# rchikhi/rust-seq2kminmers

Measured on AMD Instinct MI355X. Metric: input bases/s (Gbp/s) for k-min-mer extraction, l=31 k=10 d=0.01, higher is better.
Workload: dtype u32

## Files before the change

### rust-seq2kminmers_amd/csrc/s2k_api.hip

```cpp
#include "../../include/s2k.h"
#include "s2k_dev.h"
#include "s2k_hostcopy.h"

#include <math.h>
#include <stdio.h>
#include <stdlib.h>
#include <string.h>
#include <string>
#include <algorithm>
#include <atomic>
#include <chrono>
#include <condition_variable>
#include <thread>
#include <memory>
#include <mutex>
#include <sys/mman.h>
#include <vector>

using namespace s2k;

static_assert(offsetof(Counts, path) == offsetof(s2k_counts, path), "Counts must start with s2k_counts");

namespace {

// ... 516 lines not shown
                                  use_desc ? (unsigned long long *)d_agg : nullptr, agg_pack(0, 0, 0, 0, true, true), sp),
                "read table kernel");
        Sem sem = c.sem;
        sem.read_runs = nullptr;
        sem.tile_heads = nullptr;
        if (want_runs) {
            if (c.full_runs) {
                S2K_TRY(launch_read_run_counts(c.d_bases, c.d_read_off, n_reads, n_bases, run_blk, run_off, run_tmp, read_runs, nullptr, sp),
                        "run count kernels");
                sem.read_runs = read_runs;
            } else {
                S2K_TRY(hipMemsetAsync(tile_heads, 0, n_tiles * sizeof(uint32_t), sp), "memset tile head words");
                sem.tile_heads = tile_heads;
            }
        }
        if (use_desc) {
            Desc dz{};
            dz.agg = d_agg;
            dz.meta = d_meta;
            dz.state = d_state;
            dz.k = c.sem.k;
            dz.spec_n = ctx->rec_per_tile_hint ? ctx->rec_per_tile_hint : 192u;
            dz.km_capacity = o.km_capacity;
            dz.mn_capacity = o.mn_capacity;
            dz.o_km_off = (unsigned long long *)o.km_off;
            dz.o_hash = (unsigned long long *)o.hash;
            dz.o_start = o.start;
            dz.o_end = o.end;
            dz.o_rev = o.rev;
            dz.o_mn_off = (unsigned long long *)mn_off;
            dz.o_mn_j = o.mn_j;
            dz.o_mn_jend = o.mn_jend;
            dz.o_mn_hash = o.mn_hash;
            dz.xor_shards = (unsigned long long *)ctx->d_xor;
            if (tm) S2K_TRY(hipEventRecord(ctx->ev[1], sp), "event");
            if (tm && n_chunks > 1) S2K_TRY(hipEventRecord(ctx->ev[3], sk), "event");
            for (uint32_t ch = 0; ch < n_chunks; ch++) {
                auto cut = [&](uint32_t i) -> uint64_t {
                    static const double tail = getenv("S2K_DESC_TAIL") ? atof(getenv("S2K_DESC_TAIL")) : 0.0;
                    if (i >= n_chunks) return n_tiles;
                    if (tail <= 0.0 || tail >= 1.0 || n_chunks < 2) return n_tiles * i / n_chunks;
                    return (uint64_t)((double)n_tiles * (1.0 - tail) * (double)i / (double)(n_chunks - 1));
                };
                const uint64_t T0 = cut(ch), T1 = cut(ch + 1);
                const bool last = ch + 1 == n_chunks;
                S2K_TRY(launch_tile_minimizers(c.d_bases, c.d_read_off, n_reads, n_bases, T1, tile_read0, sem, rec,
                                               pool_cursor + (size_t)CURSOR_WORDS * ch, nullptr, nullptr, nullptr, ctx->d_counts, &dz, T0, sp),
                        "tiled minimizer kernel");
                if (last) {
                    S2K_TRY(hipEventRecord(ctx->tiles_done, sp), "event");
                    ctx->tiles_done_valid = true;
                    if (tm) S2K_TRY(hipEventRecord(ctx->ev[2], sp), "event");
                }
                S2K_TRY(hipEventRecord(ctx->chunk_ev[ch], sp), "event");
                S2K_TRY(hipStreamWaitEvent(sk, ctx->chunk_ev[ch], 0), "stream wait");
                if (tm && n_chunks == 1) S2K_TRY(hipEventRecord(ctx->ev[3], sk), "event");
#ifdef S2K_DEBUG_KNOBS
                static const bool nokm = getenv("S2K_DEBUG_NOKM") != nullptr;
                if (nokm) continue;
#endif
                S2K_TRY(launch_desc_scan(T0, T1, dz, d_scan, ctx->d_counts, sk), "tile word scan");
                S2K_TRY(launch_desc_kminmers(T0, T1, n_tiles, n_reads, dz, rec, ctx->d_counts, sk, last && !(chained && c.sem.hpc)), "k-min-mer kernel");
            }
            if (tm) S2K_TRY(hipEventRecord(ctx->ev[4], sk), "event");
            S2K_TRY(launch_finalize(ctx->d_counts, ctx->d_xor, (const uint64_t *)&d_state[n_tiles].gmn, (const uint64_t *)&d_state[n_tiles].g,
                                    o.km_capacity, o.mn_capacity, sk),
                    "finalize kernel");
            S2K_TRY(hipMemcpyAsync(ctx->h_counts, ctx->d_counts, sizeof(Counts), hipMemcpyDeviceToHost, sk), "counts copy");
            if (tm) S2K_TRY(hipEventRecord(ctx->ev[5], sk), "event");
            S2K_TRY(mark_done(ctx), "event");
            ctx->pending = true;
            return S2K_OK;
        }
        if (tm) S2K_TRY(hipEventRecord(ctx->ev[1], sp), "event");
        S2K_TRY(launch_tile_minimizers(c.d_bases, c.d_read_off, n_reads, n_bases, n_tiles, tile_read0, sem, rec, pool_cursor,
                                       tile_rec_off, tile_cnt, mn_cnt, ctx->d_counts, nullptr, 0, sp),
                "tiled minimizer kernel");
        s2k_status hs = hand_over();
        if (hs != S2K_OK) return hs;
        S2K_TRY(launch_scan_u32(tile_cnt, n_tiles, tile_goff, scan_tmp, 0, sk), "scan");
        S2K_TRY(launch_scan_u32(mn_cnt, n_reads, mn_off, scan_tmp, 0, sk), "scan");
    }
    S2K_TRY(launch_scan_u32(mn_cnt, n_reads, o.km_off, scan_tmp, c.sem.k, sk), "scan");
    if (tm) S2K_TRY(hipEventRecord(ctx->ev[3], sk), "event");
    S2K_TRY(launch_kminmers(n_tiles, tile_rec_off, tile_cnt, tile_goff, rec, mn_off, o.km_off, c.sem.k, o.km_capacity, o.hash,
                            o.start, o.end, o.rev, o.mn_capacity, o.mn_capacity ? o.mn_j : nullptr, o.mn_jend, o.mn_hash,
                            ctx->d_xor, ctx->d_counts, sk),
            "k-min-mer kernel");
    if (tm) S2K_TRY(hipEventRecord(ctx->ev[4], sk), "event");
    S2K_TRY(launch_finalize(ctx->d_counts, ctx->d_xor, mn_off + n_reads, o.km_off + n_reads, o.km_capacity, o.mn_capacity, sk),
// ... 808 lines not shown
```

### rust-seq2kminmers_amd/csrc/s2k_dev.h

```cpp
#pragma once
#include <hip/hip_runtime.h>
#include <stdint.h>

namespace s2k {

constexpr uint32_t SEED_A = 0x95c60474u, SEED_C = 0x62a02b4cu, SEED_G = 0x82572324u, SEED_T = 0x4be24456u;

__host__ __device__ inline uint32_t seed_h_scalar(uint32_t c) {
    return c == 'A' ? SEED_A : c == 'C' ? SEED_C : c == 'G' ? SEED_G : c == 'T' ? SEED_T : c == 'N' ? 0u : 1u;
}
__host__ __device__ inline uint32_t seed_rc_scalar(uint32_t c) {
    return c == 'A' ? SEED_T : c == 'C' ? SEED_G : c == 'G' ? SEED_C : c == 'T' ? SEED_A : c == 'N' ? 0u : 1u;
}
__host__ __device__ inline uint32_t seed_h_simd(uint32_t c) {
    uint32_t n = c & 15u;
    return n == 1 ? SEED_A : n == 3 ? SEED_C : n == 7 ? SEED_G : n == 4 ? SEED_T : 0u;
}
__host__ __device__ inline uint32_t seed_rc_simd(uint32_t c) {
    uint32_t n = c & 15u;
    return n == 1 ? SEED_T : n == 3 ? SEED_G : n == 7 ? SEED_C : n == 4 ? SEED_A : 0u;
}

#if defined(__HIP_DEVICE_COMPILE__)
__device__ __forceinline__ uint32_t xor3(uint32_t a, uint32_t b, uint32_t c) {
// ... 20 lines not shown
struct Sem {
    uint32_t l;
    uint32_t k;
    uint32_t bound_le;
    uint32_t enabled;
    uint32_t hpc;
    uint32_t simd_seeds;
    uint32_t keep_last;
    uint32_t end_kind;
    uint32_t tail_quirk;
    uint32_t dbg_skip;
    uint32_t pad_;
    const uint32_t *read_runs;
    uint32_t *tile_heads;
};

struct Counts {
    uint64_t n_reads, n_bases, n_minimizers, n_kminmers, xor_hash;
    uint32_t hash_bound, path;
    uint64_t pool_needed;
    uint32_t pool_overflow, bad_input, km_overflow, mn_overflow;
    uint32_t need_legacy, need_runs;
    uint64_t dbg_cycles[64][16];
#ifdef S2K_DEBUG_KNOBS
    uint64_t dbg_wave[4096][2];
#endif
};

constexpr uint32_t HW_VALID = 1u << 31, HW_PASS = 1u << 30, HW_COUNT = 0xFFFFu;

// ... 133 lines not shown

hipError_t launch_serial_count(const uint8_t *bases, const uint64_t *read_off, uint64_t n_reads, uint64_t n_bases, Sem sem,
                               uint32_t *mn_cnt, hipStream_t st);
hipError_t launch_serial_write(const uint8_t *bases, const uint64_t *read_off, uint64_t n_reads, uint64_t n_bases, Sem sem,
                               const uint64_t *mn_off, Records rec, Counts *counts, hipStream_t st);

hipError_t launch_kminmers(uint64_t n_tiles, const uint64_t *tile_rec_off, const uint32_t *tile_cnt,
                           const uint64_t *tile_goff, Records rec, const uint64_t *mn_off, const uint64_t *km_off,
                           uint32_t k, uint64_t km_capacity, uint64_t *o_hash, uint32_t *o_start, uint32_t *o_end,
                           uint8_t *o_rev, uint64_t mn_capacity, uint32_t *o_mn_j, uint32_t *o_mn_jend,
                           uint32_t *o_mn_hash, uint64_t *xor_shards, const Counts *counts, hipStream_t st);
hipError_t launch_finalize(Counts *counts, const uint64_t *xor_shards, const uint64_t *mn_total, const uint64_t *km_total,
                           uint64_t km_capacity, uint64_t mn_capacity, hipStream_t st);

hipError_t launch_tile_minimizers(const uint8_t *bases, const uint64_t *read_off, uint64_t n_reads, uint64_t n_bases,
                                  uint64_t n_tiles, const uint32_t *tile_read0, Sem sem, Records rec,
                                  uint64_t *pool_cursor, uint64_t *tile_rec_off, uint32_t *tile_cnt, uint32_t *mn_cnt,
                                  Counts *counts, const Desc *desc, uint64_t tile_begin, hipStream_t st);
hipError_t launch_desc_scan(uint64_t tile_begin, uint64_t tile_end, Desc dz, unsigned long long *scan_tmp ,
                            const Counts *counts, hipStream_t st);
size_t desc_scan_tmp_words(uint64_t n_tiles);
hipError_t launch_desc_kminmers(uint64_t tile_begin, uint64_t tile_end, uint64_t n_tiles, uint64_t n_reads, Desc dz, Records rec, Counts *counts,
                                hipStream_t st, bool alone);

hipError_t launch_hpc_count(const uint8_t *bases, const uint64_t *read_off, uint64_t n_reads, uint32_t *run_cnt, hipStream_t st,
                            bool rle = false);
hipError_t launch_hpc_write(const uint8_t *bases, const uint64_t *read_off, uint64_t n_reads, const uint64_t *hpc_off,
                            uint8_t *o_hpc, uint32_t *o_pos, uint64_t capacity, hipStream_t st, bool rle = false);

size_t fx_ws_bytes(uint64_t n);
hipError_t fx_parse_count(const uint8_t *d_raw, uint64_t n, int fastq, void *ws, uint64_t *d_totals, hipStream_t st);
// ... 5 lines not shown
```

### rust-seq2kminmers_amd/csrc/s2k_tile.hip

```cpp
#include "s2k_tile_impl.h"

namespace s2k {

#define S2K_DECL(LV)                                                                                                     \
    hipError_t launch_tiles_static_##LV(bool hpc, hipStream_t st, const uint8_t *bases, const uint64_t *read_off,         \
                                        uint64_t n_reads, uint64_t n_bases, uint64_t n_tiles, const uint32_t *tile_read0, \
                                        Sem sem, Records rec, uint64_t *pool_cursor, uint64_t *tile_rec_off,             \
                                        uint32_t *tile_cnt, uint32_t *mn_cnt, Counts *counts, const Desc *desc, uint64_t tile_begin);
S2K_STATIC_LS(S2K_DECL)
#undef S2K_DECL


hipError_t launch_tile_minimizers(const uint8_t *bases, const uint64_t *read_off, uint64_t n_reads, uint64_t n_bases,
                                  uint64_t n_tiles, const uint32_t *tile_read0, Sem sem, Records rec,
                                  uint64_t *pool_cursor, uint64_t *tile_rec_off, uint32_t *tile_cnt, uint32_t *mn_cnt,
                                  Counts *counts, const Desc *desc, uint64_t tile_begin, hipStream_t st) {
    if (n_tiles <= tile_begin || n_reads == 0) return hipSuccess;
    if (sem.l > (uint32_t)MAX_L_TILED || (sem.hpc && sem.tail_quirk && !sem.read_runs && !sem.tile_heads)) return hipErrorInvalidValue;
    if (desc && (desc->k == 0 || desc->k > 32u || !desc->agg || !desc->meta)) return hipErrorInvalidValue;
    switch (sem.l) {
#define S2K_CASE(LV)                                                                                                   \
    case LV:                                                                                                           \
        return launch_tiles_static_##LV(sem.hpc, st, bases, read_off, n_reads, n_bases, n_tiles, tile_read0, sem, rec, \
                                        pool_cursor, tile_rec_off, tile_cnt, mn_cnt, counts, desc, tile_begin);
        S2K_STATIC_LS(S2K_CASE)
#undef S2K_CASE
    default:
        return launch_tiles_l<0>(sem.hpc, st, bases, read_off, n_reads, n_bases, n_tiles, tile_read0, sem, rec,
                                 pool_cursor, tile_rec_off, tile_cnt, mn_cnt, counts, desc, tile_begin);
    }
}

}
```

### rust-seq2kminmers_amd/csrc/s2k_tile_impl.h

```cpp
#pragma once
#include "s2k_dev.h"
#include "s2k_static_l.h"

#include <cstdlib>
#include <mutex>
#include <type_traits>

namespace s2k {
namespace {

#ifndef S2K_TW
#define S2K_TW 12
#endif
#ifndef S2K_TW_REG
#ifdef S2K_PROFILE
#define S2K_TW_REG 12
#else
#define S2K_TW_REG 16
#endif
#endif
template <bool HPC> constexpr int tw() { return HPC ? S2K_TW : S2K_TW_REG; }
template <bool HPC> constexpr int waves_per_simd() { return tw<HPC>() / 4; }
static_assert(S2K_TW % 4 == 0 && S2K_TW_REG % 4 == 0, "whole waves per SIMD");
constexpr int HS_OFF = 16;
// ... 1061 lines not shown
                        f ^= rotl32(ti.x, l - 1 - i);
                        r ^= rotr32(ti.y, l - 1 - i);
                    }
                }
            }
            f ^= (uint32_t)__builtin_amdgcn_update_dpp(0, (int)f, 0xB1, 0xf, 0xf, false);
            r ^= (uint32_t)__builtin_amdgcn_update_dpp(0, (int)r, 0xB1, 0xf, 0xf, false);
            f ^= (uint32_t)__builtin_amdgcn_update_dpp(0, (int)f, 0x4E, 0xf, 0xf, false);
            r ^= (uint32_t)__builtin_amdgcn_update_dpp(0, (int)r, 0x4E, 0xf, 0xf, false);
            if (act && part == 0) rec.hash[base + S.jobslot[job]] = f < r ? f : r;
        }
        njobs = 0;
        wave_sync();
    };
    auto batch = [&](uint32_t b0, auto single_c) {
        constexpr bool SINGLE = decltype(single_c)::value;
        wave_sync();
        bool listed = false;
        if constexpr (HPC && SINGLE && S2K_LPH != 0) {
            if (Tq <= 112u) {
                listed = true;
                typedef __attribute__((address_space(3))) uint8_t lds_b;
                typedef __attribute__((address_space(3))) uint32_t lds_w;
                typedef uint32_t u32x2 __attribute__((ext_vector_type(2)));
                typedef uint32_t u32x4 __attribute__((ext_vector_type(4)));
                typedef __attribute__((address_space(3))) u32x2 lds_w2;
                typedef __attribute__((address_space(3))) u32x4 lds_w4;
                constexpr uint32_t XT = TILE_BASES + 128 - 2048;
                static_assert(XT % 16 == 0 && XT >= 7168 + MAX_L_TILED + 16 && LISTCAP <= 192, "the tables of the listing must not reach into the compacted tile");
                const uint32_t dq = (uint32_t)(uintptr_t)(lds_b *)const_cast<uint8_t *>(D) + XT;
// ... 62 lines not shown
#pragma unroll
            for (int d = 0; d < 5; d++) {
                uint32_t wv = vm[d];
                const uint32_t rw = raw[d];
                constexpr int CPW = 32 / CAPP;
                auto capw = [&](int i) { return caps[(CPW * d + i) < NPC ? CPW * d + i : NPC - 1]; };
                const uint32_t cap0 = capw(0), cap1 = capw(1), cap2 = capw(CPW > 2 ? 2 : 0), cap3 = capw(CPW > 2 ? 3 : 1);
                while (wv) {
                    const uint32_t bit = __builtin_ctz(wv);
                    wv &= wv - 1;
                    const uint32_t pm = CAPP == 16 ? (0xFFFFu << (bit & 16)) : (0xFFu << (bit & 24));
                    const uint32_t later = rw & (pm & ~((2u << bit) - 1u));
                    const uint32_t hvk = CAPP == 16 ? ((bit & 16) ? cap1 : cap0) : ((bit & 16) ? ((bit & 8) ? cap3 : cap2) : ((bit & 8) ? cap1 : cap0));
                    if (SINGLE || (k >= b0 && k < b0 + LISTCAP)) {
                        S.list[k - b0] = (uint16_t)((tql + 32 * d + bit) | (later ? 0x8000u : 0u));
                        if (!later && !(sem.dbg_skip & 16)) rec.hash[base + k] = hvk;
                    }
                    k++;
                }
            }
        }
        wave_sync();
        S2K_STAMP(4);
        const uint32_t bn = N - b0 < (uint32_t)LISTCAP ? N - b0 : (uint32_t)LISTCAP;
        for (uint32_t k0 = 0; k0 < bn; k0 += 64) {
            const uint32_t kq = k0 + lane;
            const uint32_t e = kq < bn ? S.list[kq] : 0u;
            const bool need = (e & 0x8000u) != 0;
            uint64_t jobs = __ballot(need);
#ifdef S2K_PROFILE
            if ((sem.dbg_skip & 8) && lane == 0) ph[7] += (uint64_t)__popcll(jobs);
// ... 33 lines not shown
        for (uint32_t k0 = 0; k0 < bn; k0 += 64) {
            asm volatile("; S2K_MARK round_begin many=%0" ::"i"(MANY ? 1 : 0));
            const uint32_t kk = k0 + lane;
            const bool act = kk < bn;
            uint32_t x = 0, rid = 0;
            uint32_t prel = 0, erel = 0;
            if (act) x = S.list[kk] & 0x3FFFu;
            S2K_STAMP(8);
            if (act) backmap(x, prel, erel);
            S2K_STAMP(9);
            if constexpr (DESC) {
                if (act) {
                    const uint32_t span = erel - prel;
                    if (span > (uint32_t)REC_SPAN_MAX) counts->need_legacy = 1;
                    const uint32_t sp = span > (uint32_t)REC_SPAN_MAX ? (uint32_t)REC_SPAN_MAX : span;
                    if (!(sem.dbg_skip & 16)) rec.j[base + b0 + kk] = prel | (sp << 14);
                }
            } else {
            const uint64_t p = t0 + prel, e1 = t0 + erel;
            if (act) {
                uint64_t rstart;
                if constexpr (!MANY) {
                    uint32_t c = 0;
                    for (uint32_t i = 0; i < nb; i++) c += (S.hb[i] <= (int32_t)x);
                    rid = r0 + c;
                    rstart = c == 0 ? rs0 : t0 + S.rs16[c];
                } else {
                    uint32_t lo = r0, hi = r1;
                    while (lo < hi) {
                        uint32_t mid = lo + (hi - lo + 1) / 2;
                        if (read_off[mid] <= p) lo = mid;
                        else hi = mid - 1;
                    }
                    rid = lo;
                    rstart = read_off[lo];
                }
                const uint64_t slot = base + b0 + kk;
                if (!(sem.dbg_skip & 16)) {
                    rec.j[slot] = (uint32_t)(p - rstart);
                    rec.jend[slot] = (uint32_t)(e1 - rstart);
                    rec.rid[slot] = rid;
                }
            }
            S2K_STAMP(10);
            if constexpr (MANY) {
                uint64_t remm = __ballot(act);
                while (remm) {
                    const int z = __builtin_ctzll(remm);
                    const uint32_t rz = bcast(rid, z);
                    const uint64_t same = __ballot(act && rid == rz);
                    if (lane == z) atomicAdd(&mn_cnt[rz], (uint32_t)__popcll(same));
                    remm &= ~same;
                }
            }
            }
            asm volatile("; S2K_MARK round_end many=%0" ::"i"(MANY ? 1 : 0));
        }
        };
        if constexpr (DESC) {
            rounds(std::false_type{});
        } else {
            if (many) rounds(std::true_type{});
            else rounds(std::false_type{});
        }
    };
    if (N <= (uint32_t)LISTCAP) batch(0u, std::true_type{});
    else
        for (uint32_t b0 = 0; b0 < N; b0 += LISTCAP) batch(b0, std::false_type{});
    return N;
}

template <int L, bool HPC, bool DESC>
__global__ __launch_bounds__(64 * tw<HPC>(), waves_per_simd<HPC>()) void tile_minimizer_kernel(
    const uint8_t *__restrict__ bases, const uint64_t *__restrict__ read_off, uint64_t n_reads, uint64_t n_bases,
    uint64_t n_tiles, const uint32_t *__restrict__ tile_read0, Sem sem, Records rec, uint64_t *pool_cursor,
    uint64_t *__restrict__ tile_rec_off, uint32_t *__restrict__ tile_cnt, uint32_t *mn_cnt, Counts *counts,
    unsigned long long *__restrict__ d_agg, TileMeta *__restrict__ d_meta, uint32_t K1, uint64_t tile_begin) {
    extern __shared__ __attribute__((aligned(16))) uint8_t smem[];
    using WL = WaveLdsT<HPC>;
    uint2 *tab = reinterpret_cast<uint2 *>(smem);
    if ((uint32_t)(uintptr_t)(__attribute__((address_space(3))) uint8_t *)smem != 0u) __builtin_trap();
    const int lane0 = threadIdx.x & 63, w = __builtin_amdgcn_readfirstlane((int)(threadIdx.x >> 6));
    int lane = lane0;
    const uint32_t l = L > 0 ? (uint32_t)L : sem.l;
    constexpr int TW = tw<HPC>();
    for (int c = threadIdx.x; c < 256; c += 64 * TW) {
        uint32_t cc = c;
        uint32_t h = sem.simd_seeds ? seed_h_simd(cc) : seed_h_scalar(cc), r = sem.simd_seeds ? seed_rc_simd(cc) : seed_rc_scalar(cc);
        tab[c] = make_uint2(h, rotl32(r, l - 1));
        tab[256 + c] = make_uint2(rotl32(h, l), rotr32(r, 1));
    }
    if constexpr (HPC && S2K_WARM2 != 0)
        for (int c = threadIdx.x; c < 256; c += 64 * TW) {
            const uint32_t cc = c;
            const uint32_t h = sem.simd_seeds ? seed_h_simd(cc) : seed_h_scalar(cc), r = sem.simd_seeds ? seed_rc_simd(cc) : seed_rc_scalar(cc);
            reinterpret_cast<uint2 *>(smem + WARM_OFF)[c] = make_uint2(rotl32(h, 1), rotr32(rotl32(r, l - 1), 1));
        }
    if constexpr (HPC && S2K_SEL8 != 0)
        for (int c = threadIdx.x; c < 256 * 8; c += 64 * TW) {
            const uint32_t m = (uint32_t)c >> 3, n = (uint32_t)c & 7u;
            smem[SEL8_OFF + c] = (uint8_t)(n < (uint32_t)__popc(m) ? select_nth_32(m, n) : 0x0Cu);
        }
    __syncthreads();
#ifdef S2K_DEBUG_KNOBS
    const uint64_t dbg_mt0 = __builtin_amdgcn_s_memtime(), dbg_rt0 = __builtin_amdgcn_s_memrealtime();
#endif
    WL &S = *reinterpret_cast<WL *>(smem + table_bytes<HPC>() + (size_t)w * sizeof(WL));
    uint8_t *D = S.buf + HS_OFF;
    const uint64_t n_waves = (uint64_t)gridDim.x * TW;
    uint64_t t = tile_begin + (uint64_t)blockIdx.x * TW + w;
    if (t >= n_tiles) return;
    if (__builtin_amdgcn_readfirstlane((int)counts->bad_input)) return;
    uint64_t stamp = __builtin_amdgcn_s_memtime();
#ifdef S2K_PROFILE
    ph_ptr_t ph = reinterpret_cast<ph_ptr_t>((uint32_t)(table_bytes<HPC>() + TW * sizeof(WL) + (size_t)w * 128));
    if (lane0 < 16) ph[lane0] = 0;
    wave_sync();
#else
    ph_ptr_t ph = nullptr;
#endif

    auto is_full = [&](uint64_t tt) { return (tt + 1) * (uint64_t)TILE_BASES + 128 <= n_bases; };
    uint32_t prevb = 0;
    bool have_pre = false;
    typedef __attribute__((address_space(3))) uint8_t lds_u8s;
    auto prefetch = [&](uint64_t tt) {
        static_assert(NPRE == 10, "4 + 4 + 1 wave-wide loads of 1 KiB and one of 128 B");
// ... 12 lines not shown
        }
        const uint8_t *pg = g + 8192;
        const uint32_t m = (uint32_t)__builtin_amdgcn_readfirstlane((int)(lbase + 8192u));
        asm volatile("s_mov_b32 %0, m0\n\ts_mov_b32 m0, %2\n\ts_nop 0\n\tglobal_load_lds_dwordx4 %1, off\n\ts_mov_b32 m0, %0"
                     : "=&s"(save) : "v"(pg), "s"(m) : "memory");
        if (lane < 8)
            asm volatile("s_mov_b32 %0, m0\n\ts_mov_b32 m0, %2\n\ts_nop 0\n\tglobal_load_lds_dwordx4 %1, off offset:1024\n\ts_mov_b32 m0, %0"
                         : "=&s"(save) : "v"(pg), "s"(m) : "memory");
    };
    auto byte_before = [&](uint64_t tt) -> uint32_t { return tt > 0 ? (uint32_t)bases[tt * (uint64_t)TILE_BASES - 1] : 0u; };
    auto read_entries = [&](uint32_t rr0, uint64_t &bp, uint64_t &rs) {
        const uint64_t bri = (uint64_t)rr0 + 1 + lane;
        bp = bri <= n_reads ? read_off[bri] : ~0ull;
        rs = read_off[rr0];
    };
    uint32_t r0 = tile_read0[t], r1 = tile_read0[t + 1];
    uint64_t bpos0, rs0;
    read_entries(r0, bpos0, rs0);
    if (is_full(t)) prevb = byte_before(t);
    __builtin_amdgcn_s_waitcnt(0x0F70);
    if (is_full(t)) {
        prefetch(t);
        have_pre = true;
    }
    uint32_t stores_after_dma = 0;
    uint64_t tn = t + n_waves, tnn = t + 2 * n_waves;
    const uint64_t dyn0 = tile_begin + 3 * n_waves;
    const uint32_t cur_g = (uint32_t)((blockIdx.x * TW + w + blockIdx.x / (TILE_CURSORS / 4)) % TILE_CURSORS);
    unsigned int *const cursors = (unsigned int *)(pool_cursor + 16);
    uint32_t r0n = 0, r1n = 0;
    if (tn < n_tiles) {
        r0n = tile_read0[tn];
        r1n = tile_read0[tn + 1];
    }

    uint32_t prio_iter = 0;
    bool lb_dead = sem.tile_heads != nullptr && __builtin_amdgcn_readfirstlane((int)counts->need_runs) != 0;
    for (; t < n_tiles;) {
        lane = lane0;
        asm volatile("" : "+v"(lane));
        if (sem.tile_heads) {
            switch ((prio_iter++ + (uint32_t)(w >> 2)) % 3u) {
                case 0: __builtin_amdgcn_s_setprio(0); break;
                case 1: __builtin_amdgcn_s_setprio(1); break;
                default: __builtin_amdgcn_s_setprio(2); break;
            }
        }
        const uint64_t t0 = t * (uint64_t)TILE_BASES;
        const uint64_t rem = n_bases - t0;
        const uint32_t avail = rem > (uint64_t)(TILE_BASES + 128) ? (uint32_t)(TILE_BASES + 128) : (uint32_t)rem;
        const uint32_t tile_len = rem > (uint64_t)TILE_BASES ? (uint32_t)TILE_BASES : (uint32_t)rem;
        uint32_t l16_tile = 16 * lane;
        if (__builtin_amdgcn_readfirstlane((int)have_pre)) {
            constexpr int SPR = stores_per_round<DESC>();
            asm volatile("; S2K_MARK counted_wait per_round=%0" ::"i"(SPR));
// ... 16 lines not shown
                uint4 v = make_uint4(0, 0, 0, 0);
                if (off + 16 <= avail) {
                    v = *reinterpret_cast<const uint4 *>(g + off);
                } else if (off < avail) {
                    uint32_t tmp[4] = {0, 0, 0, 0};
                    for (uint32_t b = 0; off + b < avail && b < 16; b++) tmp[b >> 2] |= (uint32_t)g[off + b] << (8 * (b & 3));
                    v = make_uint4(tmp[0], tmp[1], tmp[2], tmp[3]);
                }
                *reinterpret_cast<uint4 *>(D + off) = v;
            }
            prevb = t0 > 0 ? (uint32_t)bases[t0 - 1] : 0u;
            __builtin_amdgcn_s_waitcnt(0x0F70);
        }
        const uint32_t cr0 = r0, cr1 = r1, cprev = prevb;
        uint32_t took = 0;
        if (lane == 0 && tnn < n_tiles) took = atomicAdd(&cursors[32 * cur_g], 1u);
        uint64_t bposn = ~0ull, rs0n = 0;
        uint32_t r0nn = 0, r1nn = 0, prevbn = 0;
        const uint64_t brin = (uint64_t)r0n + 1 + lane;
        uint32_t vzero = 0;
        asm volatile("" : "+v"(vzero));
        if (tn < n_tiles) {
            bposn = read_off[brin <= n_reads ? brin : n_reads];
            rs0n = read_off[(uint64_t)r0n + vzero];
            prevbn = (uint32_t)bases[tn * (uint64_t)TILE_BASES - 1 + vzero];
            if (tnn < n_tiles) {
                r0nn = tile_read0[tnn + vzero];
                r1nn = tile_read0[tnn + 1 + vzero];
            }
        }
        if (lane == 0) S.buf[HS_OFF - 1] = 0;
        if constexpr (HPC) {
            uint2 *rz = reinterpret_cast<uint2 *>(&S.row[lane][0]);
            rz[0] = make_uint2(0u, 0u);
            rz[1] = make_uint2(0u, 0u);
            S.row[lane][4] = 0;
        }
        wave_sync();
        S2K_STAMP(0);

        uint32_t nh = tile_len;
        uint32_t lb_early = 0;
        uint32_t halo_n = 0;
// ... 14 lines not shown
                    else
                        last_start = read_off[cr1];
                }
                publish_tile_heads(sem.tile_heads, t, S, nh, t0, tile_len, ns != 0, last_start, t0 == 0 || rs0 == t0, lane);
                if (!(t0 == 0 || rs0 == t0) && t >= 1 + (uint64_t)lane)
                    lb_early = __hip_atomic_load(sem.tile_heads + (t - 1 - (uint64_t)lane), __ATOMIC_RELAXED, __HIP_MEMORY_SCOPE_AGENT);
            }
            const int need = (int)((nh + 1023) >> 10);
            np = need <= 1 ? 1 : need <= 3 ? 3 : need <= 5 ? 5 : need <= 7 ? 7 : 9;
            rcpTq = need <= 1 ? 65537u : need <= 3 ? 21846u : need <= 5 ? 13108u : need <= 7 ? 9363u : 7282u;
        }
        S2K_STAMP(1);
        auto issue_next = [&](uint32_t n_rec, uint64_t rec_base) {
            if constexpr (!DESC) {
                if (lane == 0) {
                    tile_cnt[t] = n_rec;
                    tile_rec_off[t] = rec_base;
                }
            }
            have_pre = false;
            if (tn < n_tiles && is_full(tn)) {
                prefetch(tn);
                have_pre = true;
            }
        };
        const uint32_t Tq = 16 * np;
        uint32_t N = 0;
        uint64_t base = 0;
        uint32_t caps[NPC], raw[5];
#pragma unroll
        for (int g2 = 0; g2 < NPC; g2++) caps[g2] = 0;
#pragma unroll
// ... 43 lines not shown
        prevbn = (uint32_t)__builtin_amdgcn_readfirstlane((int)prevbn);
        uint64_t drawn = ~0ull;
        if (tnn < n_tiles)
            drawn = dyn0 + cur_g + (uint64_t)TILE_CURSORS * (uint32_t)__builtin_amdgcn_readfirstlane((int)took);
        bool issued = false;
        auto issue_once = [&](uint32_t n_rec, uint64_t rec_base) {
            if (!issued) issue_next(n_rec, rec_base);
            issued = true;
        };
        int lane_d = lane;
        asm volatile("" : "+v"(lane_d));
        if (DESC || (nh != 0 && sem.enabled)) {
#ifndef EXP_NODENSE
            if (!(sem.dbg_skip & 2))
                N = dense_phase<L, HPC, DESC>(issue_once, S, D, tab, read_off, n_reads, t, t0, tile_len, nh, halo_n, Tq, rcpTq, l, cr0, cr1,
                                           bpos0, rs0, lane_d, rec, pool_cursor, mn_cnt, counts, base, sem, d_agg, d_meta, K1,
                                           caps, raw, lb_early, lb_dead, ph, stamp);
#endif
            S2K_STAMP(5);
        }
        issue_once(0, 0);
        {
            const bool many = (cr1 - cr0) > (uint32_t)(NBL - 2) || (sem.dbg_skip & 16) != 0;
            constexpr uint32_t LISTCAP = (uint32_t)listcap<HPC>();
            const uint32_t last = N == 0 ? 0u : N - ((N - 1) / LISTCAP) * LISTCAP;
            stores_after_dma = many ? 0u : (uint32_t)stores_per_round<DESC>() * ((last + 63u) / 64u);
        }
        wave_sync();
        r0 = r0n; r1 = r1n; bpos0 = bposn; rs0 = rs0n; r0n = r0nn; r1n = r1nn; prevb = prevbn;
        t = tn;
        tn = tnn;
        if (tnn < n_tiles) tnn = drawn;
        S2K_STAMP(6);
    }
#ifdef S2K_PROFILE
    if ((sem.dbg_skip & 8) && lane == 0)
        for (int i = 0; i < 16; i++) atomicAdd((unsigned long long *)&counts->dbg_cycles[blockIdx.x & 63][i], (unsigned long long)ph[i]);
#endif
#ifdef S2K_DEBUG_KNOBS
    if ((sem.dbg_skip & 32) && lane == 0) {
        const unsigned long long now = __builtin_amdgcn_s_memrealtime();
        atomicMax((unsigned long long *)&counts->dbg_cycles[0][0], now);
        atomicMax((unsigned long long *)&counts->dbg_cycles[0][1], ~now);
        atomicAdd((unsigned long long *)&counts->dbg_cycles[1][0], (unsigned long long)(__builtin_amdgcn_s_memtime() - dbg_mt0));
        atomicAdd((unsigned long long *)&counts->dbg_cycles[1][1], (unsigned long long)(now - dbg_rt0));
        const uint32_t wid = blockIdx.x * TW + w;
        if (wid < 4096) {
            counts->dbg_wave[wid][0] = now;
            counts->dbg_wave[wid][1] = ((uint64_t)__builtin_amdgcn_s_getreg((20 | (0 << 6) | (31 << 11))) << 32) | (uint32_t)__builtin_amdgcn_s_getreg((4 | (0 << 6) | (31 << 11)));
        }
    }
#endif
}

#ifndef S2K_STREAM_BUILD
#define S2K_STREAM_BUILD 0
#endif
#if S2K_STREAM_BUILD
#ifndef S2K_STREAM_DEFAULT
#define S2K_STREAM_DEFAULT 0
#endif
#ifndef S2K_STREAM_TW
#define S2K_STREAM_TW 16
#endif
// ... 126 lines not shown
            S2K_HIP_CHECK(hipGetDeviceProperties(&prop, dev));
            n_cu_d[dev] = prop.multiProcessorCount;
        }
        uint64_t blocks = (n_tiles_full - tile_begin + STREAM_TW - 1) / STREAM_TW;
        const uint64_t resident = (uint64_t)n_cu_d[dev] * STREAM_BPC;
        if (blocks > resident) blocks = resident;
        hipLaunchKernelGGL(kern, dim3((unsigned)blocks), dim3(64 * STREAM_TW), lds, st, bases, read_off, n_reads, n_bases, n_tiles_full, tile_read0, sem, rec,
                           pool_cursor, counts, desc->agg, desc->meta, desc->k - 1u, tile_begin);
        return hipGetLastError();
    } else {
        return hipErrorInvalidValue;
    }
}
#endif

template <int L, bool HPC, bool DESC>
hipError_t launch_tiles_lh(hipStream_t st, const uint8_t *bases, const uint64_t *read_off, uint64_t n_reads, uint64_t n_bases,
                           uint64_t n_tiles, const uint32_t *tile_read0, Sem sem, Records rec, uint64_t *pool_cursor,
                           uint64_t *tile_rec_off, uint32_t *tile_cnt, uint32_t *mn_cnt, Counts *counts, const Desc *desc, uint64_t tile_begin) {
    auto kern = tile_minimizer_kernel<L, HPC, DESC>;
    constexpr int TW = tw<HPC>();
    const int lds = block_lds_bytes<HPC>();
    constexpr int MAX_DEV = 64;
    static int n_cu_d[MAX_DEV] = {0}, per_cu_d[MAX_DEV] = {0};
    static std::mutex cache_mu;
    int dev = 0;
    S2K_HIP_CHECK(hipGetDevice(&dev));
    if (dev < 0 || dev >= MAX_DEV) return hipErrorInvalidDevice;
    std::lock_guard<std::mutex> lk(cache_mu);
    if (n_cu_d[dev] == 0) {
        S2K_HIP_CHECK(hipFuncSetAttribute(reinterpret_cast<const void *>(kern), hipFuncAttributeMaxDynamicSharedMemorySize, lds));
        hipDeviceProp_t prop;
        S2K_HIP_CHECK(hipGetDeviceProperties(&prop, dev));
        int occ = 0;
        S2K_HIP_CHECK(hipOccupancyMaxActiveBlocksPerMultiprocessor(&occ, reinterpret_cast<const void *>(kern), 64 * TW, lds));
        const int fit = (int)((size_t)prop.sharedMemPerMultiprocessor / (((size_t)lds + 2047) & ~(size_t)2047));
        if (fit >= 1 && occ > fit) occ = fit;
        per_cu_d[dev] = occ < 1 ? 1 : occ;
#ifdef S2K_DEBUG_KNOBS
        if (const char *e = getenv("S2K_DEBUG_BLOCKS_PER_CU")) per_cu_d[dev] = atoi(e) > 0 ? atoi(e) : per_cu_d[dev];
#endif
        n_cu_d[dev] = prop.multiProcessorCount;
    }
    const int n_cu = n_cu_d[dev], per_cu = per_cu_d[dev];
    uint64_t blocks = (n_tiles - tile_begin + TW - 1) / TW;
    const uint64_t resident = (uint64_t)n_cu * per_cu;
    if (blocks > resident) blocks = resident;
    hipLaunchKernelGGL(kern, dim3((unsigned)blocks), dim3(64 * TW), lds, st, bases, read_off, n_reads, n_bases, n_tiles,
                       tile_read0, sem, rec, pool_cursor, tile_rec_off, tile_cnt, mn_cnt, counts, desc ? desc->agg : nullptr,
                       desc ? desc->meta : nullptr, desc ? desc->k - 1u : 0u, tile_begin);
    return hipGetLastError();
}

template <int L>
hipError_t launch_tiles_l(bool hpc, hipStream_t st, const uint8_t *bases, const uint64_t *read_off, uint64_t n_reads,
                          uint64_t n_bases, uint64_t n_tiles, const uint32_t *tile_read0, Sem sem, Records rec,
                          uint64_t *pool_cursor, uint64_t *tile_rec_off, uint32_t *tile_cnt, uint32_t *mn_cnt,
                          Counts *counts, const Desc *desc, uint64_t tile_begin) {
#define S2K_GO(H, F)                                                                                                       \
    launch_tiles_lh<L, H, F>(st, bases, read_off, n_reads, n_bases, n_tiles, tile_read0, sem, rec, pool_cursor, tile_rec_off, \
                             tile_cnt, mn_cnt, counts, desc, tile_begin)
#if S2K_STREAM_BUILD
    if constexpr (L > 0) {
        static const bool use_stream = S2K_STREAM_DEFAULT ? !(getenv("S2K_STREAM_KERNEL") && atoi(getenv("S2K_STREAM_KERNEL")) == 0)
                                                          : (getenv("S2K_STREAM_KERNEL") && atoi(getenv("S2K_STREAM_KERNEL")) != 0);
        if (desc && !hpc && use_stream) {
            const uint64_t n_full = n_bases >= 128 ? (n_bases - 128) / (uint64_t)TILE_BASES : 0;
            const uint64_t hi = n_full < n_tiles ? n_full : n_tiles;
            if (hi > tile_begin) {
                S2K_HIP_CHECK(launch_stream_l<L>(st, bases, read_off, n_reads, n_bases, hi, tile_read0, sem, rec, pool_cursor, counts, desc, tile_begin));
                if (hi >= n_tiles) return hipSuccess;
                const uint64_t tb = hi;
                return launch_tiles_lh<L, false, true>(st, bases, read_off, n_reads, n_bases, n_tiles, tile_read0, sem, rec, pool_cursor, tile_rec_off, tile_cnt,
                                                       mn_cnt, counts, desc, tb);
            }
        }
    }
#endif
    if (desc) return hpc ? S2K_GO(true, true) : S2K_GO(false, true);
    return hpc ? S2K_GO(true, false) : S2K_GO(false, false);
#undef S2K_GO
}

}
}
```

### rust-seq2kminmers_amd/csrc/s2k_tile_inst.hip

```cpp
#ifndef S2K_TILE_L
#error "compile with -DS2K_TILE_L=<l>"
#endif
#include "s2k_tile_impl.h"

namespace s2k {

#define S2K_NAME2(LV) launch_tiles_static_##LV
#define S2K_NAME(LV) S2K_NAME2(LV)
hipError_t S2K_NAME(S2K_TILE_L)(bool hpc, hipStream_t st, const uint8_t *bases, const uint64_t *read_off, uint64_t n_reads,
                                uint64_t n_bases, uint64_t n_tiles, const uint32_t *tile_read0, Sem sem, Records rec,
                                uint64_t *pool_cursor, uint64_t *tile_rec_off, uint32_t *tile_cnt, uint32_t *mn_cnt,
                                Counts *counts, const Desc *desc, uint64_t tile_begin) {
    static_assert(S2K_TILE_L >= 1 && S2K_TILE_L <= 32, "the unrolled loop keeps one address register per base of the l-mer");
    return launch_tiles_l<S2K_TILE_L>(hpc, st, bases, read_off, n_reads, n_bases, n_tiles, tile_read0, sem, rec, pool_cursor,
                                      tile_rec_off, tile_cnt, mn_cnt, counts, desc, tile_begin);
}

}
```

Before: 1788.

## Specialize tile kernel on semantic mode and reload cold args from kernarg segment

Adds a compile-time tile mode (regular/HPC/runtime) so the minimizer kernel can constant-fold semantic flags such as keep_last, end_kind, simd_seeds and the debug-skip bits when the configuration matches a common case. Rarely used pointers are moved into a TileCold struct that is re-read through the kernarg segment pointer on demand rather than held live in scalar registers. Record array pointers are also hoisted into locals, and asm barriers pin a few values in SGPRs. The aim is to cut SGPR/VGPR pressure and branching in the hot loop. In exchange it doubles the kernel instantiations and relies on kernarg-segment layout tricks.

```diff
diff --git a/rust-seq2kminmers_amd/csrc/s2k_api.hip b/rust-seq2kminmers_amd/csrc/s2k_api.hip
--- a/rust-seq2kminmers_amd/csrc/s2k_api.hip
+++ b/rust-seq2kminmers_amd/csrc/s2k_api.hip
@@ -554,6 +554,7 @@
                 sem.tile_heads = tile_heads;
             }
         }
+        const uint32_t tile_mode = tile_mode_of(sem);
         if (use_desc) {
             Desc dz{};
             dz.agg = d_agg;
@@ -584,7 +585,7 @@
                 };
                 const uint64_t T0 = cut(ch), T1 = cut(ch + 1);
                 const bool last = ch + 1 == n_chunks;
-                S2K_TRY(launch_tile_minimizers(c.d_bases, c.d_read_off, n_reads, n_bases, T1, tile_read0, sem, rec,
+                S2K_TRY(launch_tile_minimizers(c.d_bases, c.d_read_off, n_reads, n_bases, T1, tile_read0, sem, tile_mode, rec,
                                                pool_cursor + (size_t)CURSOR_WORDS * ch, nullptr, nullptr, nullptr, ctx->d_counts, &dz, T0, sp),
                         "tiled minimizer kernel");
                 if (last) {
@@ -613,7 +614,7 @@
             return S2K_OK;
         }
         if (tm) S2K_TRY(hipEventRecord(ctx->ev[1], sp), "event");
-        S2K_TRY(launch_tile_minimizers(c.d_bases, c.d_read_off, n_reads, n_bases, n_tiles, tile_read0, sem, rec, pool_cursor,
+        S2K_TRY(launch_tile_minimizers(c.d_bases, c.d_read_off, n_reads, n_bases, n_tiles, tile_read0, sem, tile_mode, rec, pool_cursor,
                                        tile_rec_off, tile_cnt, mn_cnt, ctx->d_counts, nullptr, 0, sp),
                 "tiled minimizer kernel");
         s2k_status hs = hand_over();
diff --git a/rust-seq2kminmers_amd/csrc/s2k_dev.h b/rust-seq2kminmers_amd/csrc/s2k_dev.h
--- a/rust-seq2kminmers_amd/csrc/s2k_dev.h
+++ b/rust-seq2kminmers_amd/csrc/s2k_dev.h
@@ -58,6 +58,14 @@
     const uint32_t *read_runs;
     uint32_t *tile_heads;
 };
+
+enum TileMode : uint32_t { TILE_MODE_RUNTIME = 0, TILE_MODE_REGULAR = 1, TILE_MODE_HPC = 2 };
+__host__ __device__ inline uint32_t tile_mode_of(const Sem &s) {
+    if (s.enabled != 1 || s.simd_seeds || s.tail_quirk || s.read_runs || s.tile_heads) return TILE_MODE_RUNTIME;
+    if (!s.hpc && s.keep_last == 1 && s.end_kind == 0) return TILE_MODE_REGULAR;
+    if (s.hpc == 1 && s.keep_last == 0 && s.end_kind == 1) return TILE_MODE_HPC;
+    return TILE_MODE_RUNTIME;
+}
 
 struct Counts {
     uint64_t n_reads, n_bases, n_minimizers, n_kminmers, xor_hash;
@@ -221,7 +229,7 @@
                            uint64_t km_capacity, uint64_t mn_capacity, hipStream_t st);
 
 hipError_t launch_tile_minimizers(const uint8_t *bases, const uint64_t *read_off, uint64_t n_reads, uint64_t n_bases,
-                                  uint64_t n_tiles, const uint32_t *tile_read0, Sem sem, Records rec,
+                                  uint64_t n_tiles, const uint32_t *tile_read0, Sem sem, uint32_t mode, Records rec,
                                   uint64_t *pool_cursor, uint64_t *tile_rec_off, uint32_t *tile_cnt, uint32_t *mn_cnt,
                                   Counts *counts, const Desc *desc, uint64_t tile_begin, hipStream_t st);
 hipError_t launch_desc_scan(uint64_t tile_begin, uint64_t tile_end, Desc dz, unsigned long long *scan_tmp ,
diff --git a/rust-seq2kminmers_amd/csrc/s2k_tile.hip b/rust-seq2kminmers_amd/csrc/s2k_tile.hip
--- a/rust-seq2kminmers_amd/csrc/s2k_tile.hip
+++ b/rust-seq2kminmers_amd/csrc/s2k_tile.hip
@@ -5,28 +5,29 @@
 #define S2K_DECL(LV)                                                                                                     \
     hipError_t launch_tiles_static_##LV(bool hpc, hipStream_t st, const uint8_t *bases, const uint64_t *read_off,         \
                                         uint64_t n_reads, uint64_t n_bases, uint64_t n_tiles, const uint32_t *tile_read0, \
-                                        Sem sem, Records rec, uint64_t *pool_cursor, uint64_t *tile_rec_off,             \
+                                        Sem sem, uint32_t mode, Records rec, uint64_t *pool_cursor, uint64_t *tile_rec_off, \
                                         uint32_t *tile_cnt, uint32_t *mn_cnt, Counts *counts, const Desc *desc, uint64_t tile_begin);
 S2K_STATIC_LS(S2K_DECL)
 #undef S2K_DECL
 
 
 hipError_t launch_tile_minimizers(const uint8_t *bases, const uint64_t *read_off, uint64_t n_reads, uint64_t n_bases,
-                                  uint64_t n_tiles, const uint32_t *tile_read0, Sem sem, Records rec,
+                                  uint64_t n_tiles, const uint32_t *tile_read0, Sem sem, uint32_t mode, Records rec,
                                   uint64_t *pool_cursor, uint64_t *tile_rec_off, uint32_t *tile_cnt, uint32_t *mn_cnt,
                                   Counts *counts, const Desc *desc, uint64_t tile_begin, hipStream_t st) {
     if (n_tiles <= tile_begin || n_reads == 0) return hipSuccess;
     if (sem.l > (uint32_t)MAX_L_TILED || (sem.hpc && sem.tail_quirk && !sem.read_runs && !sem.tile_heads)) return hipErrorInvalidValue;
     if (desc && (desc->k == 0 || desc->k > 32u || !desc->agg || !desc->meta)) return hipErrorInvalidValue;
+    if (mode != TILE_MODE_RUNTIME && mode != tile_mode_of(sem)) return hipErrorInvalidValue;
     switch (sem.l) {
 #define S2K_CASE(LV)                                                                                                   \
     case LV:                                                                                                           \
-        return launch_tiles_static_##LV(sem.hpc, st, bases, read_off, n_reads, n_bases, n_tiles, tile_read0, sem, rec, \
+        return launch_tiles_static_##LV(sem.hpc, st, bases, read_off, n_reads, n_bases, n_tiles, tile_read0, sem, mode, rec, \
                                         pool_cursor, tile_rec_off, tile_cnt, mn_cnt, counts, desc, tile_begin);
         S2K_STATIC_LS(S2K_CASE)
 #undef S2K_CASE
     default:
-        return launch_tiles_l<0>(sem.hpc, st, bases, read_off, n_reads, n_bases, n_tiles, tile_read0, sem, rec,
+        return launch_tiles_l<0>(sem.hpc, st, bases, read_off, n_reads, n_bases, n_tiles, tile_read0, sem, mode, rec,
                                  pool_cursor, tile_rec_off, tile_cnt, mn_cnt, counts, desc, tile_begin);
     }
 }
diff --git a/rust-seq2kminmers_amd/csrc/s2k_tile_impl.h b/rust-seq2kminmers_amd/csrc/s2k_tile_impl.h
--- a/rust-seq2kminmers_amd/csrc/s2k_tile_impl.h
+++ b/rust-seq2kminmers_amd/csrc/s2k_tile_impl.h
@@ -1099,6 +1099,7 @@
         wave_sync();
     };
     auto batch = [&](uint32_t b0, auto single_c) {
+        uint32_t *const rec_j = rec.j, *const rec_hash = rec.hash, *const rec_jend = rec.jend, *const rec_rid = rec.rid;
         constexpr bool SINGLE = decltype(single_c)::value;
         wave_sync();
         bool listed = false;
@@ -1191,7 +1192,7 @@
                     const uint32_t hvk = CAPP == 16 ? ((bit & 16) ? cap1 : cap0) : ((bit & 16) ? ((bit & 8) ? cap3 : cap2) : ((bit & 8) ? cap1 : cap0));
                     if (SINGLE || (k >= b0 && k < b0 + LISTCAP)) {
                         S.list[k - b0] = (uint16_t)((tql + 32 * d + bit) | (later ? 0x8000u : 0u));
-                        if (!later && !(sem.dbg_skip & 16)) rec.hash[base + k] = hvk;
+                        if (!later && !(sem.dbg_skip & 16)) rec_hash[base + k] = hvk;
                     }
                     k++;
                 }
@@ -1255,7 +1256,7 @@
                     const uint32_t span = erel - prel;
                     if (span > (uint32_t)REC_SPAN_MAX) counts->need_legacy = 1;
                     const uint32_t sp = span > (uint32_t)REC_SPAN_MAX ? (uint32_t)REC_SPAN_MAX : span;
-                    if (!(sem.dbg_skip & 16)) rec.j[base + b0 + kk] = prel | (sp << 14);
+                    if (!(sem.dbg_skip & 16)) rec_j[base + b0 + kk] = prel | (sp << 14);
                 }
             } else {
             const uint64_t p = t0 + prel, e1 = t0 + erel;
@@ -1278,9 +1279,9 @@
                 }
                 const uint64_t slot = base + b0 + kk;
                 if (!(sem.dbg_skip & 16)) {
-                    rec.j[slot] = (uint32_t)(p - rstart);
-                    rec.jend[slot] = (uint32_t)(e1 - rstart);
-                    rec.rid[slot] = rid;
+                    rec_j[slot] = (uint32_t)(p - rstart);
+                    rec_jend[slot] = (uint32_t)(e1 - rstart);
+                    rec_rid[slot] = rid;
                 }
             }
             S2K_STAMP(10);
@@ -1311,12 +1312,46 @@
     return N;
 }
 
-template <int L, bool HPC, bool DESC>
+template <int MODE>
+__device__ __forceinline__ Sem tile_sem(Sem s) {
+#ifndef S2K_DEBUG_KNOBS
+    s.dbg_skip = 0;
+#endif
+    if constexpr (MODE != TILE_MODE_RUNTIME) {
+        s.enabled = 1;
+        s.hpc = MODE == TILE_MODE_HPC;
+        s.simd_seeds = 0;
+        s.keep_last = MODE == TILE_MODE_HPC ? 0 : 1;
+        s.end_kind = MODE == TILE_MODE_HPC ? 1 : 0;
+        s.tail_quirk = 0;
+        s.read_runs = nullptr;
+        s.tile_heads = nullptr;
+    }
+    return s;
+}
+
+struct TileCold {
+    Records rec;
+    uint64_t *pool_cursor;
+    uint64_t *tile_rec_off;
+    uint32_t *tile_cnt;
+    uint32_t *mn_cnt;
+    Counts *counts;
+    unsigned long long *d_agg;
+    TileMeta *d_meta;
+    const uint32_t *tile_read0;
+    uint32_t K1;
+};
+typedef const __attribute__((address_space(4))) TileCold *cold_ptr_t;
+
+template <int L, bool HPC, bool DESC, int MODE>
 __global__ __launch_bounds__(64 * tw<HPC>(), waves_per_simd<HPC>()) void tile_minimizer_kernel(
-    const uint8_t *__restrict__ bases, const uint64_t *__restrict__ read_off, uint64_t n_reads, uint64_t n_bases,
-    uint64_t n_tiles, const uint32_t *__restrict__ tile_read0, Sem sem, Records rec, uint64_t *pool_cursor,
-    uint64_t *__restrict__ tile_rec_off, uint32_t *__restrict__ tile_cnt, uint32_t *mn_cnt, Counts *counts,
-    unsigned long long *__restrict__ d_agg, TileMeta *__restrict__ d_meta, uint32_t K1, uint64_t tile_begin) {
+    const TileCold cold, const uint8_t *__restrict__ bases, const uint64_t *__restrict__ read_off, uint64_t n_reads,
+    uint64_t n_bases, uint64_t n_tiles, Sem sem_arg, uint64_t tile_begin) {
+    const Sem sem = tile_sem<MODE>(sem_arg);
+    (void)cold;
+    cold_ptr_t cold_p = (cold_ptr_t)__builtin_amdgcn_kernarg_segment_ptr();
+    auto cold_args = [&]() -> const TileCold & { return *(const TileCold *)cold_p; };
     extern __shared__ __attribute__((aligned(16))) uint8_t smem[];
     using WL = WaveLdsT<HPC>;
     uint2 *tab = reinterpret_cast<uint2 *>(smem);
@@ -1346,12 +1381,12 @@
 #ifdef S2K_DEBUG_KNOBS
     const uint64_t dbg_mt0 = __builtin_amdgcn_s_memtime(), dbg_rt0 = __builtin_amdgcn_s_memrealtime();
 #endif
-    WL &S = *reinterpret_cast<WL *>(smem + table_bytes<HPC>() + (size_t)w * sizeof(WL));
-    uint8_t *D = S.buf + HS_OFF;
+    uint32_t wl_off = (uint32_t)(table_bytes<HPC>() + (size_t)w * sizeof(WL));
+    uint8_t *D = reinterpret_cast<WL *>(smem + wl_off)->buf + HS_OFF;
     const uint64_t n_waves = (uint64_t)gridDim.x * TW;
     uint64_t t = tile_begin + (uint64_t)blockIdx.x * TW + w;
     if (t >= n_tiles) return;
-    if (__builtin_amdgcn_readfirstlane((int)counts->bad_input)) return;
+    if (__builtin_amdgcn_readfirstlane((int)cold_args().counts->bad_input)) return;
     uint64_t stamp = __builtin_amdgcn_s_memtime();
 #ifdef S2K_PROFILE
     ph_ptr_t ph = reinterpret_cast<ph_ptr_t>((uint32_t)(table_bytes<HPC>() + TW * sizeof(WL) + (size_t)w * 128));
@@ -1394,7 +1429,7 @@
         bp = bri <= n_reads ? read_off[bri] : ~0ull;
         rs = read_off[rr0];
     };
-    uint32_t r0 = tile_read0[t], r1 = tile_read0[t + 1];
+    uint32_t r0 = cold_args().tile_read0[t], r1 = cold_args().tile_read0[t + 1];
     uint64_t bpos0, rs0;
     read_entries(r0, bpos0, rs0);
     if (is_full(t)) prevb = byte_before(t);
@@ -1407,18 +1442,23 @@
     uint64_t tn = t + n_waves, tnn = t + 2 * n_waves;
     const uint64_t dyn0 = tile_begin + 3 * n_waves;
     const uint32_t cur_g = (uint32_t)((blockIdx.x * TW + w + blockIdx.x / (TILE_CURSORS / 4)) % TILE_CURSORS);
-    unsigned int *const cursors = (unsigned int *)(pool_cursor + 16);
+    auto cursors = [&]() { return (unsigned int *)(cold_args().pool_cursor + 16); };
     uint32_t r0n = 0, r1n = 0;
     if (tn < n_tiles) {
-        r0n = tile_read0[tn];
-        r1n = tile_read0[tn + 1];
+        r0n = cold_args().tile_read0[tn];
+        r1n = cold_args().tile_read0[tn + 1];
     }
 
     uint32_t prio_iter = 0;
-    bool lb_dead = sem.tile_heads != nullptr && __builtin_amdgcn_readfirstlane((int)counts->need_runs) != 0;
+    bool lb_dead = sem.tile_heads != nullptr && __builtin_amdgcn_readfirstlane((int)cold_args().counts->need_runs) != 0;
     for (; t < n_tiles;) {
         lane = lane0;
         asm volatile("" : "+v"(lane));
+        asm volatile("" : "+s"(cold_p));
+        asm volatile("" : "+s"(bases));
+        asm volatile("" : "+s"(wl_off));
+        WL &S = *reinterpret_cast<WL *>(smem + wl_off);
+        D = S.buf + HS_OFF;
         if (sem.tile_heads) {
             switch ((prio_iter++ + (uint32_t)(w >> 2)) % 3u) {
                 case 0: __builtin_amdgcn_s_setprio(0); break;
@@ -1465,7 +1505,7 @@
         }
         const uint32_t cr0 = r0, cr1 = r1, cprev = prevb;
         uint32_t took = 0;
-        if (lane == 0 && tnn < n_tiles) took = atomicAdd(&cursors[32 * cur_g], 1u);
+        if (lane == 0 && tnn < n_tiles) took = atomicAdd(&cursors()[32 * cur_g], 1u);
         uint64_t bposn = ~0ull, rs0n = 0;
         uint32_t r0nn = 0, r1nn = 0, prevbn = 0;
         const uint64_t brin = (uint64_t)r0n + 1 + lane;
@@ -1476,8 +1516,8 @@
             rs0n = read_off[(uint64_t)r0n + vzero];
             prevbn = (uint32_t)bases[tn * (uint64_t)TILE_BASES - 1 + vzero];
             if (tnn < n_tiles) {
-                r0nn = tile_read0[tnn + vzero];
-                r1nn = tile_read0[tnn + 1 + vzero];
+                r0nn = cold_args().tile_read0[tnn + vzero];
+                r1nn = cold_args().tile_read0[tnn + 1 + vzero];
             }
         }
         if (lane == 0) S.buf[HS_OFF - 1] = 0;
@@ -1522,8 +1562,8 @@
         auto issue_next = [&](uint32_t n_rec, uint64_t rec_base) {
             if constexpr (!DESC) {
                 if (lane == 0) {
-                    tile_cnt[t] = n_rec;
-                    tile_rec_off[t] = rec_base;
+                    cold_args().tile_cnt[t] = n_rec;
+                    cold_args().tile_rec_off[t] = rec_base;
                 }
             }
             have_pre = false;
@@ -1597,7 +1637,8 @@
 #ifndef EXP_NODENSE
             if (!(sem.dbg_skip & 2))
                 N = dense_phase<L, HPC, DESC>(issue_once, S, D, tab, read_off, n_reads, t, t0, tile_len, nh, halo_n, Tq, rcpTq, l, cr0, cr1,
-                                           bpos0, rs0, lane_d, rec, pool_cursor, mn_cnt, counts, base, sem, d_agg, d_meta, K1,
+                                           bpos0, rs0, lane_d, cold_args().rec, cold_args().pool_cursor, cold_args().mn_cnt,
+                                           cold_args().counts, base, sem, cold_args().d_agg, cold_args().d_meta, cold_args().K1,
                                            caps, raw, lb_early, lb_dead, ph, stamp);
 #endif
             S2K_STAMP(5);
@@ -1618,19 +1659,19 @@
     }
 #ifdef S2K_PROFILE
     if ((sem.dbg_skip & 8) && lane == 0)
-        for (int i = 0; i < 16; i++) atomicAdd((unsigned long long *)&counts->dbg_cycles[blockIdx.x & 63][i], (unsigned long long)ph[i]);
+        for (int i = 0; i < 16; i++) atomicAdd((unsigned long long *)&cold_args().counts->dbg_cycles[blockIdx.x & 63][i], (unsigned long long)ph[i]);
 #endif
 #ifdef S2K_DEBUG_KNOBS
     if ((sem.dbg_skip & 32) && lane == 0) {
         const unsigned long long now = __builtin_amdgcn_s_memrealtime();
-        atomicMax((unsigned long long *)&counts->dbg_cycles[0][0], now);
-        atomicMax((unsigned long long *)&counts->dbg_cycles[0][1], ~now);
-        atomicAdd((unsigned long long *)&counts->dbg_cycles[1][0], (unsigned long long)(__builtin_amdgcn_s_memtime() - dbg_mt0));
-        atomicAdd((unsigned long long *)&counts->dbg_cycles[1][1], (unsigned long long)(now - dbg_rt0));
+        atomicMax((unsigned long long *)&cold_args().counts->dbg_cycles[0][0], now);
+        atomicMax((unsigned long long *)&cold_args().counts->dbg_cycles[0][1], ~now);
+        atomicAdd((unsigned long long *)&cold_args().counts->dbg_cycles[1][0], (unsigned long long)(__builtin_amdgcn_s_memtime() - dbg_mt0));
+        atomicAdd((unsigned long long *)&cold_args().counts->dbg_cycles[1][1], (unsigned long long)(now - dbg_rt0));
         const uint32_t wid = blockIdx.x * TW + w;
         if (wid < 4096) {
-            counts->dbg_wave[wid][0] = now;
-            counts->dbg_wave[wid][1] = ((uint64_t)__builtin_amdgcn_s_getreg((20 | (0 << 6) | (31 << 11))) << 32) | (uint32_t)__builtin_amdgcn_s_getreg((4 | (0 << 6) | (31 << 11)));
+            cold_args().counts->dbg_wave[wid][0] = now;
+            cold_args().counts->dbg_wave[wid][1] = ((uint64_t)__builtin_amdgcn_s_getreg((20 | (0 << 6) | (31 << 11))) << 32) | (uint32_t)__builtin_amdgcn_s_getreg((4 | (0 << 6) | (31 << 11)));
         }
     }
 #endif
@@ -1787,11 +1828,11 @@
 }
 #endif
 
-template <int L, bool HPC, bool DESC>
+template <int L, bool HPC, bool DESC, int MODE>
 hipError_t launch_tiles_lh(hipStream_t st, const uint8_t *bases, const uint64_t *read_off, uint64_t n_reads, uint64_t n_bases,
                            uint64_t n_tiles, const uint32_t *tile_read0, Sem sem, Records rec, uint64_t *pool_cursor,
                            uint64_t *tile_rec_off, uint32_t *tile_cnt, uint32_t *mn_cnt, Counts *counts, const Desc *desc, uint64_t tile_begin) {
-    auto kern = tile_minimizer_kernel<L, HPC, DESC>;
+    auto kern = tile_minimizer_kernel<L, HPC, DESC, MODE>;
     constexpr int TW = tw<HPC>();
     const int lds = block_lds_bytes<HPC>();
     constexpr int MAX_DEV = 64;
@@ -1819,20 +1860,32 @@
     uint64_t blocks = (n_tiles - tile_begin + TW - 1) / TW;
     const uint64_t resident = (uint64_t)n_cu * per_cu;
     if (blocks > resident) blocks = resident;
-    hipLaunchKernelGGL(kern, dim3((unsigned)blocks), dim3(64 * TW), lds, st, bases, read_off, n_reads, n_bases, n_tiles,
-                       tile_read0, sem, rec, pool_cursor, tile_rec_off, tile_cnt, mn_cnt, counts, desc ? desc->agg : nullptr,
-                       desc ? desc->meta : nullptr, desc ? desc->k - 1u : 0u, tile_begin);
+    TileCold cold{};
+    cold.rec = rec;
+    cold.pool_cursor = pool_cursor;
+    cold.tile_rec_off = tile_rec_off;
+    cold.tile_cnt = tile_cnt;
+    cold.mn_cnt = mn_cnt;
+    cold.counts = counts;
+    cold.d_agg = desc ? desc->agg : nullptr;
+    cold.d_meta = desc ? desc->meta : nullptr;
+    cold.tile_read0 = tile_read0;
+    cold.K1 = desc ? desc->k - 1u : 0u;
+    hipLaunchKernelGGL(kern, dim3((unsigned)blocks), dim3(64 * TW), lds, st, cold, bases, read_off, n_reads, n_bases, n_tiles, sem,
+                       tile_begin);
     return hipGetLastError();
 }
 
 template <int L>
 hipError_t launch_tiles_l(bool hpc, hipStream_t st, const uint8_t *bases, const uint64_t *read_off, uint64_t n_reads,
-                          uint64_t n_bases, uint64_t n_tiles, const uint32_t *tile_read0, Sem sem, Records rec,
+                          uint64_t n_bases, uint64_t n_tiles, const uint32_t *tile_read0, Sem sem, uint32_t mode, Records rec,
                           uint64_t *pool_cursor, uint64_t *tile_rec_off, uint32_t *tile_cnt, uint32_t *mn_cnt,
                           Counts *counts, const Desc *desc, uint64_t tile_begin) {
-#define S2K_GO(H, F)                                                                                                       \
-    launch_tiles_lh<L, H, F>(st, bases, read_off, n_reads, n_bases, n_tiles, tile_read0, sem, rec, pool_cursor, tile_rec_off, \
-                             tile_cnt, mn_cnt, counts, desc, tile_begin)
+#define S2K_GO_M(H, F, M)                                                                                                    \
+    launch_tiles_lh<L, H, F, M>(st, bases, read_off, n_reads, n_bases, n_tiles, tile_read0, sem, rec, pool_cursor,         \
+                                tile_rec_off, tile_cnt, mn_cnt, counts, desc, tile_begin)
+#define S2K_GO(H, F) \
+    (mode != TILE_MODE_RUNTIME ? S2K_GO_M(H, F, H ? TILE_MODE_HPC : TILE_MODE_REGULAR) : S2K_GO_M(H, F, TILE_MODE_RUNTIME))
 #if S2K_STREAM_BUILD
     if constexpr (L > 0) {
         static const bool use_stream = S2K_STREAM_DEFAULT ? !(getenv("S2K_STREAM_KERNEL") && atoi(getenv("S2K_STREAM_KERNEL")) == 0)
@@ -1844,8 +1897,11 @@
                 S2K_HIP_CHECK(launch_stream_l<L>(st, bases, read_off, n_reads, n_bases, hi, tile_read0, sem, rec, pool_cursor, counts, desc, tile_begin));
                 if (hi >= n_tiles) return hipSuccess;
                 const uint64_t tb = hi;
-                return launch_tiles_lh<L, false, true>(st, bases, read_off, n_reads, n_bases, n_tiles, tile_read0, sem, rec, pool_cursor, tile_rec_off, tile_cnt,
-                                                       mn_cnt, counts, desc, tb);
+                if (mode != TILE_MODE_RUNTIME)
+                    return launch_tiles_lh<L, false, true, TILE_MODE_REGULAR>(st, bases, read_off, n_reads, n_bases, n_tiles, tile_read0, sem, rec,
+                                                                              pool_cursor, tile_rec_off, tile_cnt, mn_cnt, counts, desc, tb);
+                return launch_tiles_lh<L, false, true, TILE_MODE_RUNTIME>(st, bases, read_off, n_reads, n_bases, n_tiles, tile_read0, sem, rec, pool_cursor,
+                                                                          tile_rec_off, tile_cnt, mn_cnt, counts, desc, tb);
             }
         }
     }
@@ -1853,7 +1909,8 @@
     if (desc) return hpc ? S2K_GO(true, true) : S2K_GO(false, true);
     return hpc ? S2K_GO(true, false) : S2K_GO(false, false);
 #undef S2K_GO
-}
-
-}
-}
+#undef S2K_GO_M
+}
+
+}
+}
diff --git a/rust-seq2kminmers_amd/csrc/s2k_tile_inst.hip b/rust-seq2kminmers_amd/csrc/s2k_tile_inst.hip
--- a/rust-seq2kminmers_amd/csrc/s2k_tile_inst.hip
+++ b/rust-seq2kminmers_amd/csrc/s2k_tile_inst.hip
@@ -8,11 +8,11 @@
 #define S2K_NAME2(LV) launch_tiles_static_##LV
 #define S2K_NAME(LV) S2K_NAME2(LV)
 hipError_t S2K_NAME(S2K_TILE_L)(bool hpc, hipStream_t st, const uint8_t *bases, const uint64_t *read_off, uint64_t n_reads,
-                                uint64_t n_bases, uint64_t n_tiles, const uint32_t *tile_read0, Sem sem, Records rec,
+                                uint64_t n_bases, uint64_t n_tiles, const uint32_t *tile_read0, Sem sem, uint32_t mode, Records rec,
                                 uint64_t *pool_cursor, uint64_t *tile_rec_off, uint32_t *tile_cnt, uint32_t *mn_cnt,
                                 Counts *counts, const Desc *desc, uint64_t tile_begin) {
     static_assert(S2K_TILE_L >= 1 && S2K_TILE_L <= 32, "the unrolled loop keeps one address register per base of the l-mer");
-    return launch_tiles_l<S2K_TILE_L>(hpc, st, bases, read_off, n_reads, n_bases, n_tiles, tile_read0, sem, rec, pool_cursor,
+    return launch_tiles_l<S2K_TILE_L>(hpc, st, bases, read_off, n_reads, n_bases, n_tiles, tile_read0, sem, mode, rec, pool_cursor,
                                       tile_rec_off, tile_cnt, mn_cnt, counts, desc, tile_begin);
 }
 
```

Result: faster. 1841, median of 6 (+3.0%).
